# saithepaithewhyyy/Stochastic-Gradient-MCMC-for-non-linear-state-models---MTH422

Measured on AMD Instinct MI355X. Metric: SGLD steps/sec (T=1000, N=1000 particles), higher is better.
Workload: dtype f64

## Files before the change

stochastic-gradient-mcmc-for-non-linear-state-models---mth422_amd/csrc/pfg_launch.hpp:

```cpp
#pragma once
#include <mutex>
#include "pfg_host.hpp"
#include "pfg_device.hpp"

namespace pfg_host {

#define PFG_ENSURE_LDS(ctx, kern, lds)                                                                    \
    do {                                                                                                  \
        if ((lds) > 64 * 1024) {                                                                          \
            size_t &pfg_lds_set_ = (ctx)->lds_set[reinterpret_cast<const void *>(kern)];                  \
            if ((lds) > pfg_lds_set_) {                                                                   \
                PFG_HIP(ctx, hipFuncSetAttribute(reinterpret_cast<const void *>(kern),                    \
                                                 hipFuncAttributeMaxDynamicSharedMemorySize, (int)(lds))); \
                pfg_lds_set_ = (lds);                                                                     \
            }                                                                                             \
        }                                                                                                 \
    } while (0)

constexpr int PFG_GRID_ALL = -1, PFG_GRID_INIT = -2, PFG_GRID_FINISH = -3;
template <int MODEL, int KERNEL, typename REAL, int RNG, int NT, int PPT, int KMAX>
int launch_grid_ppt(pfg_ctx *ctx, const LaunchPlan &p, int B, const pfg_dev_problem *dp, hipStream_t st) {
    constexpr int NW = NT / pfg::WAVE;
    const int phase = p.phase;
    const dim3 grid((unsigned)p.tiles, (unsigned)B), blk(NT);
// ... 40 lines not shown
    PFG_HIP(ctx, hipGetLastError());
    return PFG_OK;
}


template <int TAG>
int ensure_exp_tab_mem(pfg_ctx *ctx, hipStream_t st) {
    static std::mutex mu;
    static std::vector<char> filled;
    std::lock_guard<std::mutex> lock(mu);
    if ((size_t)ctx->device < filled.size() && filled[(size_t)ctx->device]) return PFG_OK;
    hipStreamCaptureStatus cap = hipStreamCaptureStatusNone;
    PFG_HIP(ctx, hipStreamIsCapturing(st, &cap));
    if (cap != hipStreamCaptureStatusNone)
        return fail(ctx, PFG_ERR_INVALID, "the first launch of this kernel on a device fills its exp table and cannot be captured: run one eager launch first");
    hipLaunchKernelGGL(pfg::exp_tab_mem_fill_kernel<TAG>, dim3(1), dim3(pfg::TAB_E2_ACC), 0, st);
    PFG_HIP(ctx, hipGetLastError());
    PFG_HIP(ctx, hipStreamSynchronize(st));
    if (filled.size() <= (size_t)ctx->device) filled.resize((size_t)ctx->device + 1, 0);
    filled[(size_t)ctx->device] = 1;
    return PFG_OK;
}

template <int MODEL, int KERNEL, typename REAL, int NT, int PPT, int RNG, bool PP, int MODE, bool TRACE = true, bool SCORE1 = false>
int launch_one_t(pfg_ctx *ctx, const LaunchPlan &p, int B, const pfg_dev_problem *dp, hipStream_t st) {
    using TR = pfg::RegTraits<MODEL, KERNEL, REAL, NT, PPT, RNG, PP, MODE>;
    if constexpr (TR::TABMEM) {
        if (const int rc = ensure_exp_tab_mem<TR::EXPTAB_TAG>(ctx, st)) return rc;
    }
    return launch_kernel(ctx, pfg::pf_reg_kernel<MODEL, KERNEL, REAL, NT, PPT, RNG, PP, MODE, TRACE, SCORE1>, NT, p, B, dp, st);
}
template <int MODEL, int KERNEL, typename REAL, int NT, int PPT, int RNG, bool PP>
int launch_one(pfg_ctx *ctx, const LaunchPlan &p, int B, const pfg_dev_problem *dp, hipStream_t st) {
    if constexpr (reg_score1_twin(MODEL, RNG, sizeof(REAL) == 8, NT, PPT, PP))
        if (p.score1) return launch_one_t<MODEL, KERNEL, REAL, NT, PPT, RNG, PP, pfg::MODE_PLAIN, false, true>(ctx, p, B, dp, st);
    if (!p.traced) return launch_one_t<MODEL, KERNEL, REAL, NT, PPT, RNG, PP, pfg::MODE_PLAIN, false>(ctx, p, B, dp, st);
    return launch_one_t<MODEL, KERNEL, REAL, NT, PPT, RNG, PP, pfg::MODE_PLAIN, true>(ctx, p, B, dp, st);
}
template <int MODEL, int KERNEL, typename REAL, int RNG>
int launch_v(pfg_ctx *ctx, const LaunchPlan &p, int B, const pfg_dev_problem *dp, hipStream_t st) {
#define PFG_ENTRY(NT_, PPT_, PP_)                                                                 \
    if constexpr (reg_entry_built(MODEL, RNG, sizeof(REAL) == 8, NT_, PPT_, PP_))                \
        if (p.nt == NT_ && p.ppt == PPT_ && p.pp == PP_) return launch_one<MODEL, KERNEL, REAL, NT_, PPT_, RNG, PP_>(ctx, p, B, dp, st);
    PFG_ENTRY(256, 1, true) PFG_ENTRY(256, 4, true) PFG_ENTRY(256, 4, false) PFG_ENTRY(1024, 1, true) PFG_ENTRY(64, 2, true)
    PFG_ENTRY(1024, 4, false) PFG_ENTRY(64, 4, true) PFG_ENTRY(512, 2, false)
    PFG_ENTRY(64, 2, false) PFG_ENTRY(64, 4, false)
#undef PFG_ENTRY
    return fail(ctx, PFG_ERR_INVALID, "the launch plan names no kernel of this unit");
}

template <int MODEL, int KERNEL, typename REAL, int RNG, int MODE>
// ... 88 lines not shown
```

stochastic-gradient-mcmc-for-non-linear-state-models---mth422_amd/csrc/pfg_math.hpp:

```cpp
#pragma once
#include <hip/hip_runtime.h>
#include <stdint.h>
#include <type_traits>
#include "pfgrad.h"

namespace pfg {

constexpr int WAVE = 64;
constexpr int MODE_PLAIN = 0, MODE_PARIS = 1, MODE_SYSTEMATIC = 2, MODE_N2 = 3, MODE_STRATIFIED = 4, MODE_ADAPTIVE = 5;
__host__ __device__ inline float ess_threshold_of(int32_t reserved) { return __builtin_bit_cast(float, reserved); }
constexpr double LOG_2PI = 1.8378770664093453;

template <class T> using gptr = T __attribute__((address_space(1))) *;
template <class T> __device__ __forceinline__ gptr<T> global_ptr(T *p) { return (gptr<T>)p; }

template <int CTRL>
__device__ __forceinline__ double dpp_shr0_f64(double v) {
    int lo = __builtin_amdgcn_mov_dpp(__double2loint(v), CTRL, 0xf, 0xf, true);
    int hi = __builtin_amdgcn_mov_dpp(__double2hiint(v), CTRL, 0xf, 0xf, true);
    return __hiloint2double(hi, lo);
}
template <int CTRL, int ROW_MASK>
__device__ __forceinline__ double dpp_f64(double old, double v) {
    int lo = __builtin_amdgcn_update_dpp(__double2loint(old), __double2loint(v), CTRL, ROW_MASK, 0xf, false);
// ... 295 lines not shown
    }
    template <int HOT> __device__ __forceinline__ double exp_finite_hot(double x) const {
        if constexpr (HOT == 0) return exp_tab<true>(x, t.e2); else return exp_tab_hot<true, HOT>(x, t);
    }
#endif
#else
    __device__ __forceinline__ double exp_finite(double x) const { return exp_tab(x, t.e2); }
#endif
    __device__ __forceinline__ double log(double x) const { return log_tab(x, t.lg); }
    __device__ __forceinline__ double sqrt(double x) const { return ::sqrt(x); }
    __device__ __forceinline__ double sqrt_pos(double x) const { return pfg::sqrt_pos(x); }
    __device__ __forceinline__ double rcp_pos(double x) const { return pfg::rcp_pos(x); }
    __device__ __forceinline__ void normal_pair_f32(uint32_t a, uint32_t b, float &z0, float &z1) const {
        const float u1 = ((float)a + 0.5f) * 2.3283064365386963e-10f;
        const float u2 = (float)(b >> 8) * (1.0f / 16777216.0f);
        const float r = __builtin_amdgcn_sqrtf(-1.3862943611198906f * __builtin_amdgcn_logf(u1));
        z0 = r * __builtin_amdgcn_cosf(u2);
        z1 = r * __builtin_amdgcn_sinf(u2);
    }
    __device__ __forceinline__ void normal_pair(uint32_t a, uint32_t b, double &z0, double &z1) const {
        float f0, f1;
        normal_pair_f32(a, b, f0, f1);
        z0 = (double)f0; z1 = (double)f1;
    }
};
template <> struct Math<double, false> {
    TabF64 t;
    __device__ __forceinline__ double exp(double x) const { return ::exp(x); }
    __device__ __forceinline__ double exp_acc(double x) const { return ::exp(x); }
    __device__ __forceinline__ double exp_finite(double x) const { return ::exp(x); }
    __device__ __forceinline__ double log(double x) const { return ::log(x); }
    __device__ __forceinline__ double sqrt(double x) const { return ::sqrt(x); }
    __device__ __forceinline__ double sqrt_pos(double x) const { return ::sqrt(x); }
    __device__ __forceinline__ double rcp_pos(double x) const { return 1.0 / x; }
    __device__ __forceinline__ void normal_pair(uint32_t a, uint32_t b, double &z0, double &z1) const {
        const double u1 = ((double)a + 0.5) * (1.0 / 4294967296.0);
        const double r = ::sqrt(-2.0 * ::log(u1));
        double sn, cs;
        sincospi((double)b * (1.0 / 2147483648.0), &sn, &cs);
        z0 = r * cs; z1 = r * sn;
    }
    __device__ __forceinline__ void normal_pair_f32(uint32_t a, uint32_t b, float &z0, float &z1) const {
        double d0, d1;
        normal_pair(a, b, d0, d1);
        z0 = (float)d0; z1 = (float)d1;
    }
// ... 28 lines not shown
```

stochastic-gradient-mcmc-for-non-linear-state-models---mth422_amd/csrc/pfg_reg_kernel.hpp:

```cpp
#pragma once
#include "pfg_reg_traits.hpp"

namespace pfg {

template <int NW> __device__ __forceinline__ void block_sync() {
    if (NW == 1) {
        __builtin_amdgcn_fence(__ATOMIC_RELEASE, "wavefront");
        __builtin_amdgcn_wave_barrier();
        __builtin_amdgcn_fence(__ATOMIC_ACQUIRE, "wavefront");
    } else {
        __syncthreads();
    }
}
__device__ __forceinline__ double rcp_newton2(double x) {
    double r = __builtin_amdgcn_rcp(x);
    r = fma(fma(-x, r, 1.0), r, r);
    r = fma(fma(-x, r, 1.0), r, r);
    return r;
}

template <int MODEL, int KERNEL, typename REAL, int NT, int PPT, int RNG, bool PP, int MODE = 0, bool TRACE = true, bool SCORE1 = false>
__global__ __launch_bounds__(NT) __attribute__((amdgpu_waves_per_eu(RegTraits<MODEL, KERNEL, REAL, NT, PPT, RNG, PP, MODE>::OCC_MIN, RegTraits<MODEL, KERNEL, REAL, NT, PPT, RNG, PP, MODE>::OCC_MAX))) void pf_reg_kernel(const pfg_dev_problem *__restrict__ probs) {
    using TR = RegTraits<MODEL, KERNEL, REAL, NT, PPT, RNG, PP, MODE>;
    constexpr int NS = TR::NS, H = TR::H, NW = TR::NW;
    static_assert(!TR::LWL || PP, "PaRIS / O(N^2) need the parents intact while children are built: ping-pong buffers");
    static_assert(!TR::SYSTEMATIC || RNG == PFG_RNG_DEVICE, "systematic resampling draws its offset on the device");
    extern __shared__ __align__(16) unsigned char smem[];

    const pfg_dev_problem &P = probs[blockIdx.x];
    const int N = P.N, T = P.T, t1 = P.t1, tL = P.tL;
    const int tid = threadIdx.x, lane = tid & (WAVE - 1);
    const int wave = __builtin_amdgcn_readfirstlane(tid / WAVE);
    constexpr bool ONLY_SCORE1 = PFG_EXP_PLAIN || SCORE1;
    if constexpr (SCORE1) {
        if (P.smoother != PFG_SMOOTHER_NEMETH || P.lambduh != 1.0 || P.stat != PFG_STAT_SCORE) {
            if (threadIdx.x < PFG_OUT_DOUBLES && P.out) P.out[threadIdx.x] = __builtin_nan("");
            return;
        }
    }
    if constexpr (TR::ADAPTIVE) {
        if (!(P.flags & PFG_FLAG_ADAPTIVE_RESAMPLING) || P.smoother != PFG_SMOOTHER_NEMETH || P.stat == PFG_STAT_PREDICTIVE) {
            if (threadIdx.x < PFG_OUT_DOUBLES && P.out) P.out[threadIdx.x] = __builtin_nan("");
            return;
        }
    }
    [[maybe_unused]] const double tauN = TR::ADAPTIVE ? (double)ess_threshold_of(P.reserved) * (double)N : 0.0;
    const bool is_filter = !ONLY_SCORE1 && (P.smoother == PFG_SMOOTHER_FILTER);
    const int stat = ONLY_SCORE1 ? (int)PFG_STAT_SCORE : P.stat;
    const double lam_d = ONLY_SCORE1 ? 1.0 : is_filter ? 0.0 : ((P.smoother == PFG_SMOOTHER_PARIS || TR::N2) ? 1.0 : P.lambduh);
    const REAL lam = (REAL)lam_d, oml = (REAL)(1.0 - lam_d);
    const bool needS_every = is_filter || (lam_d != 1.0);
    [[maybe_unused]] const bool raw_score = TR::RAWSCORE && !needS_every && stat == PFG_STAT_SCORE;
    const gptr<const double> yv = global_ptr(P.y);
    const gptr<const double> wv = global_ptr(P.weights);
    const gptr<const double> uv = global_ptr(P.u);
    const gptr<const double> zv = global_ptr(P.z);

    const int NLS = TR::FAST ? TR::layout(0).NLS : TR::layout(N).NLS;
    double *cdf = reg_lds_ptr<double, TR, &RegLdsLayout::cdf>(smem, N);
    uint32_t *cdfu = reg_lds_ptr<uint32_t, TR, &RegLdsLayout::cdf>(smem, N);
    REAL *cur = reg_lds_ptr<REAL, TR, &RegLdsLayout::buf0>(smem, N), *nxt = reg_lds_ptr<REAL, TR, &RegLdsLayout::buf1>(smem, N);
    auto sidx = [&](int d, int i) -> size_t { return TR::sidx(NLS, d, i); };
    double *red_scan = reg_lds_ptr<double, TR, &RegLdsLayout::red_scan>(smem, N);
    double *red_max = reg_lds_ptr<double, TR, &RegLdsLayout::red_max>(smem, N);
    float *red_maxf = reinterpret_cast<float *>(red_max);
    double *red_S = reg_lds_ptr<double, TR, &RegLdsLayout::red_S>(smem, N);
    double *red_W0 = reg_lds_ptr<double, TR, &RegLdsLayout::red_W0>(smem, N);
    const double invN = 1.0 / (double)N;
    double *tabmem = reg_lds_ptr<double, TR, &RegLdsLayout::tab>(smem, N);
    REAL *lwL = reg_lds_ptr<REAL, TR, &RegLdsLayout::lwL>(smem, N);
    int *paris_queue = reg_lds_ptr<int, TR, &RegLdsLayout::queue>(smem, N);
    int *paris_wq0 = reg_lds_ptr<int, TR, &RegLdsLayout::wq0>(smem, N), *paris_wq1 = reg_lds_ptr<int, TR, &RegLdsLayout::wq1>(smem, N);
    int *paris_Jres = reg_lds_ptr<int, TR, &RegLdsLayout::Jres>(smem, N);

    Math<REAL, TR::TAB> mth;
    mth.t.e2 = tabmem;
    mth.t.lg = reinterpret_cast<const double2 *>(tabmem + TAB_E2);
    mth.t.sc = reinterpret_cast<const double2 *>(tabmem + TAB_E2 + 2 * TAB_LG);
    if constexpr (TR::TABMEM) mth.t.e2g = (gptr<const double>)ExpTabMem<TR::EXPTAB_TAG>::e2;
    if (tab_bytes<REAL, RNG, TR::TAB>() > 0) tab_fill(tabmem, RNG == PFG_RNG_DEVICE, tid, NT);
    if (TR::FAST && !TR::BLK) {
// ... 7 lines not shown
    int np2 = 1;
    while (np2 < N) np2 <<= 1;
    if (P.stamps && tid == 0) { P.stamps[0] = __builtin_amdgcn_s_memtime(); P.stamps[1] = __builtin_amdgcn_s_memrealtime(); }
#ifdef PFG_PHASE_STAMPS
    unsigned long long ph_acc[10] = {0, 0, 0, 0, 0, 0, 0, 0, 0, 0};
    unsigned long long ph_prev = __builtin_amdgcn_s_memtime();
#define PFG_PH(i) { const unsigned long long ph_now = __builtin_amdgcn_s_memtime(); ph_acc[i] += ph_now - ph_prev; ph_prev = ph_now; }
#define PFG_MARK(s)
#elif defined(PFG_ISA_MARKERS)
#define PFG_PH(i) asm volatile("; PFG_PHASE " #i);
#define PFG_MARK(s) asm volatile("; PFG_MARK " s);
#else
#define PFG_PH(i)
#define PFG_MARK(s)
#endif

    LaneRng rng = {};
    if (RNG == PFG_RNG_DEVICE)
        rng = lane_rng_init(P.seed, P.stream, P.step_ctr ? *P.step_ctr : 0ull, (uint32_t)tid);
    auto draw_normals = [&](REAL *zz) {
#pragma unroll
        for (int k = 0; k < PPT; k += 2) {
            REAL a, b;
            mth.normal_pair(rng.next(), rng.next(), a, b);
            zz[k] = a;
            if (k + 1 < PPT) zz[k + 1] = b;
        }
    };

    REAL lw[PPT];
    long long paris_cursor = 0;
    bool paris_overflow = false;
    const bool raw = TR::RAWCAP && (P.flags & PFG_FLAG_PARIS_RAW_STREAM) != 0 && P.paris_stream != nullptr;
    bool carry_has = false;
    double *const zbuf = reinterpret_cast<double *>(paris_queue);
    long long *const raw_slots = reinterpret_cast<long long *>(red_W0 + 2);
    [[maybe_unused]] auto legacy_normals = [&]() {
        const gptr<const double> strm = global_ptr(P.paris_stream);
        const long long cap = P.paris_stream_len;
        const unsigned long long ltm = (1ull << lane) - 1ull;
        int *const wc = reinterpret_cast<int *>(red_scan);
        const int produced0 = carry_has ? 1 : 0;
        __syncthreads();
        if (carry_has && tid == 0) zbuf[0] = red_W0[1];
        const int need = (N - produced0 + 1) >> 1;
        const long long base = paris_cursor;
        int acc = 0;
// ... 118 lines not shown
    for (int h = 0; h < H; ++h) { filt[h] = 0.0; S[h] = 0.0; }
    double m = 0.0, W = (double)N;
    bool valid[PPT];
    int own[PPT];
#pragma unroll
    for (int k = 0; k < PPT; ++k) {
        valid[k] = (k * NT + tid) < N;
        own[k] = valid[k] ? (k * NT + tid) : (N - 1);
        if (!valid[k]) lw[k] = -INFINITY;
    }
    const int last = N - 1;
    [[maybe_unused]] float m_next = 0.0f;
    if constexpr (TR::STALE) {
        float ml = (float)lw[0];
#pragma unroll
        for (int k = 1; k < PPT; ++k) ml = fmaxf(ml, (float)lw[k]);
        ml = wave_max(ml);
        if (lane == 0) red_maxf[wave] = ml;
        block_sync<NW>();
        float mm = red_maxf[0];
#pragma unroll
        for (int w = 1; w < NW; ++w) mm = fmaxf(mm, red_maxf[w]);
        m = uniform_f64((double)mm);
        block_sync<NW>();
        if constexpr (TR::SHIFTFOLD) {
#pragma unroll
            for (int k = 0; k < PPT; ++k) lw[k] -= (REAL)m;
        }
    }

    for (int t = 0; t <= T; ++t) {
        [[maybe_unused]] double uu_raw[PPT];
        [[maybe_unused]] REAL zz_raw[PPT];
        if constexpr (TR::RAWCAP) {
            if (raw && t < T) {
                const gptr<const double> strm = global_ptr(P.paris_stream);
                if (paris_cursor + N > P.paris_stream_len) paris_overflow = true;
#pragma unroll
                for (int k = 0; k < PPT; ++k) uu_raw[k] = paris_overflow ? 0.5 : strm[paris_cursor + own[k]];
                if (!paris_overflow) paris_cursor += N;
                legacy_normals();
#pragma unroll
                for (int k = 0; k < PPT; ++k) zz_raw[k] = (REAL)zbuf[own[k]];
            }
        }
        [[maybe_unused]] float ml = 0.0f;
// ... 96 lines not shown
        PFG_PH(3)
        if (TR::BLK && NW == 1) {
            W = __hiloint2double(__builtin_amdgcn_readlane(__double2hiint(wave_inc), WAVE - 1),
                                 __builtin_amdgcn_readlane(__double2loint(wave_inc), WAVE - 1));
        } else if (TR::BLK) {
            const double tot = (lane < NW) ? red_scan[lane] : 0.0;
            double inc = tot;
            inc += dpp_shr0_f64<0x111>(inc);
            inc += dpp_shr0_f64<0x112>(inc);
            if (NW > 4) { inc += dpp_shr0_f64<0x114>(inc); inc += dpp_shr0_f64<0x118>(inc); }
            const double exc = inc - tot;
            const double off = __hiloint2double(__builtin_amdgcn_readlane(__double2hiint(exc), wave),
                                                __builtin_amdgcn_readlane(__double2loint(exc), wave));
#pragma unroll
            for (int k = 0; k < PPT; ++k) cs[k] += off;
            W = __hiloint2double(__builtin_amdgcn_readlane(__double2hiint(inc), NW - 1),
                                 __builtin_amdgcn_readlane(__double2loint(inc), NW - 1));
            if constexpr (TR::STALE) {
                bool retry;
                if constexpr (TR::SUMSHIFT) {
                    constexpr uint32_t W_LO = (uint32_t)(1023 - 728) << 20, W_HI = (uint32_t)(1023 + 728) << 20;
                    retry = t > 0 && !((uint32_t)__double2hiint(W) - W_LO < W_HI - W_LO);
                } else {
                    float mm = red_maxf[0];
#pragma unroll
                    for (int w = 1; w < NW; ++w) mm = fmaxf(mm, red_maxf[w]);
                    if constexpr (TR::SHIFTFOLD) mm += (float)m;
                    m_next = __builtin_bit_cast(float, __builtin_amdgcn_readfirstlane(__builtin_bit_cast(int, mm)));
                    retry = t > 0 && !(fabsf(m_next - (float)m) <= 512.0f);
                }
                if (retry) {
                    PFG_MARK("cold stale-shift-retry")
                    block_sync<NW>();
                    if constexpr (!TR::SUMSHIFT) m = uniform_f64((double)m_next);
                    const REAL y_p = (REAL)yv[t - 1], y2_p = y_p * y_p;
                    REAL lwk[PPT];
#pragma unroll
                    for (int k = 0; k < PPT; ++k) {
                        const REAL x1 = cur[sidx(0, own[k])];
                        lwk[k] = valid[k] ? svm_logw(c, x1, mth.exp_finite(-x1), y2_p) : (REAL)(-INFINITY);
                        if constexpr (!TR::SUMSHIFT) cs[k] = (double)mth.exp((REAL)(lwk[k] - (REAL)m));
                    }
                    if constexpr (TR::SUMSHIFT) {
                        float rl = (float)lwk[0];
#pragma unroll
                        for (int k = 1; k < PPT; ++k) rl = fmaxf(rl, (float)lwk[k]);
                        rl = wave_max(rl);
                        if (lane == 0) red_maxf[wave] = rl;
                        block_sync<NW>();
                        float mm = red_maxf[0];
#pragma unroll
                        for (int w = 1; w < NW; ++w) mm = fmaxf(mm, red_maxf[w]);
                        m = uniform_f64((double)mm);
#pragma unroll
                        for (int k = 0; k < PPT; ++k) cs[k] = (double)mth.exp((REAL)(lwk[k] - (REAL)m));
                    }
                    if constexpr (TR::SHIFTFOLD) {
// ... 82 lines not shown
            }
            W = uniform_f64(run);
        }
        const double invW = uniform_f64(PFG_OPT_RCPW ? rcp_newton2(W) : 1.0 / W);
        [[maybe_unused]] bool resample = true;
        if constexpr (TR::ADAPTIVE) {
            if (t < T) {
                double W2 = red_W0[4];
#pragma unroll
                for (int w = 1; w < NW; ++w) W2 += red_W0[4 + w];
                resample = __builtin_amdgcn_readfirstlane((int)(W * W < tauN * W2)) != 0;
            }
        }
        if (needS) {
            PFG_MARK("cold needS")
#pragma unroll
            for (int h = 0; h < H; ++h) {
                double acc = 0.0;
#pragma unroll
                for (int w = 0; w < NW; ++w) acc += red_S[h * NW + w];
                S[h] = uniform_f64(acc * invW);
            }
        }
        if (wave == 0) {
            PFG_MARK("w0.25 wave0-loglik")
            const bool counts = t > 0 && (t - 1) >= t1 && (t - 1) < tL;
            if (TR::LAZYLL) {
                const bool mine = lane == (t & (WAVE - 1));
                ll_W = mine ? W : ll_W;
                ll_w = mine ? (counts ? wt_prev : 0.0) : ll_w;
                ll_m = mine ? (float)m : ll_m;
                const bool due = (t & (WAVE - 1)) == WAVE - 1 || t == T;
                if (due || (!TR::TWINLESS_LL && PFG_TR(P.trace_ll))) {
                    PFG_MARK("cold loglik-flush")
                    const double term = ll_w * ((double)ll_m + (double)mth.log((REAL)(ll_W * invN)));
                    ll = uniform_f64(ll + wave_sum(term));
                    ll_w = 0.0;
                } else if (TR::TWINLESS_LL && PFG_TR(P.trace_ll)) {
                    const double term = ll_w * ((double)ll_m + (double)mth.log((REAL)(ll_W * invN)));
                    const double run = ll + wave_sum(term);
                    if (tid == 0) P.trace_ll[t] = run;
                }
                if ((due || !TR::TWINLESS_LL) && PFG_TR(P.trace_ll) && tid == 0) P.trace_ll[t] = ll;
            } else {
                if (counts) ll = uniform_f64(ll + wt_prev * (m + log(W / (double)N)));
                if (PFG_TR(P.trace_ll) && tid == 0) P.trace_ll[t] = ll;
            }
// ... 12 lines not shown
        const bool use_stat = inside && (stat != PFG_STAT_NONE);
        const bool plain = !needS_every;
        if (!TR::ADAPTIVE || resample) {
        if (TR::BLK) {
            {
                const double fixs = invW * 4294967296.0;
#pragma unroll
                for (int k = 0; k < PPT; ++k)
                    cdfu[cdf_phys(tid * PPT + k)] = cvt_u32_sat(cs[k] * fixs);
            }
        } else {
#pragma unroll
            for (int k = 0; k < PPT; ++k)
                if (valid[k]) {
                    cdf[TR::FAST ? cdf_phys(k * NT + tid) : k * NT + tid] = cs[k] * invW;
                    if (TR::PARIS || TR::N2) lwL[k * NT + tid] = lw[k];
                }
        }
        PFG_PH(4)
        block_sync<NW>();
        PFG_PH(5)
        if (TR::PRIO == 1) __builtin_amdgcn_s_setprio(2);
        if (TR::PRIO == 2) __builtin_amdgcn_s_setprio(0);

        if (RNG != PFG_RNG_REPLAY) {
            if (TR::SYSTEMATIC) {
                const double u0 = red_W0[0];
#pragma unroll
                for (int k = 0; k < PPT; ++k) uu[k] = ((double)(k * NT + tid) + u0) * invN;
                if (PFG_TR(P.trace_x) && P.rec_ud) {
#pragma unroll
                    for (int k = 0; k < PPT; ++k)
                        if (valid[k]) P.rec_ud[(size_t)t * N + k * NT + tid] = uu[k];
                }
            } else if (TR::STRATIFIED) {
#pragma unroll
                for (int k = 0; k < PPT; ++k) uu[k] = ((double)(k * NT + tid) + u01_32(rng.next())) * invN;
                if (PFG_TR(P.trace_x) && P.rec_ud) {
#pragma unroll
                    for (int k = 0; k < PPT; ++k)
                        if (valid[k]) P.rec_ud[(size_t)t * N + k * NT + tid] = uu[k];
                }
            } else if (!TR::BLK) {
#pragma unroll
                for (int k = 0; k < PPT; ++k) uu[k] = u01_32(rng.next());
                if (TR::ADAPTIVE && PFG_TR(P.trace_x) && P.rec_ud) {
// ... 6 lines not shown
#pragma unroll
            for (int k = 0; k < PPT; ++k) uu[k] = ((double)(k * NT + tid) + uu[k]) / (double)N;
        }
        }
        int anc[PPT];
        [[maybe_unused]] uint32_t gaddr[PPT];
#pragma unroll
        for (int k = 0; k < PPT; ++k) { anc[k] = 0; gaddr[k] = 0u; }
        if (!TR::ADAPTIVE || resample) {
        if (TR::BLK) {
            uint32_t ua[PPT];
#pragma unroll
            for (int k = 0; k < PPT; ++k) ua[k] = TR::SORTED ? us[k] : rng.next();
#ifdef PFG_EXP_EVENWORDS
#pragma unroll
            for (int k = 0; k < PPT; ++k) ua[k] = (uint32_t)(((uint64_t)(tid * PPT + k) << 32) / (uint64_t)(NT * PPT)) + (ua[k] >> 12);
#endif
            if (PFG_TR(P.trace_x) && P.rec_u) {
#pragma unroll
                for (int k = 0; k < PPT; ++k)
                    if (valid[k]) P.rec_u[(size_t)t * N + k * NT + tid] = ua[k];
            }
            using lds_u32 = const __attribute__((address_space(3))) uint32_t;
            const uint32_t cdf_base = (uint32_t)(uintptr_t)(lds_u32 *)cdfu;
            uint32_t off[PPT];
#pragma unroll
            for (int k = 0; k < PPT; ++k) off[k] = cdf_base;
            constexpr int FIRST_STEP = TR::PIVOTS ? 128 : (NT * PPT) >> 1;
            if constexpr (TR::PIVOTS) {
                const uint32_t p511 = __builtin_amdgcn_readfirstlane(cdfu[cdf_phys(511)]);
                const uint32_t p255 = __builtin_amdgcn_readfirstlane(cdfu[cdf_phys(255)]);
                const uint32_t p767 = __builtin_amdgcn_readfirstlane(cdfu[cdf_phys(767)]);
#pragma unroll
                for (int k = 0; k < PPT; ++k) {
                    const bool g1 = p511 <= ua[k];
                    const uint32_t t2 = g1 ? p767 : p255;
                    const bool g2 = t2 <= ua[k];
                    off[k] += (g1 ? 4u * (512 + 16) : 0u) + (g2 ? 4u * (256 + 8) : 0u);
                }
            }
#pragma unroll
            for (int step = FIRST_STEP; step >= 1; step >>= 1) {
                const int probe = step - 1 + (step >= 32 ? (step >> 5) - 1 : 0);
                const int adv = step + (step >> 5);
                uint32_t cv[PPT];
#pragma unroll
                for (int k = 0; k < PPT; ++k) cv[k] = *(lds_u32 *)(uintptr_t)(off[k] + 4u * probe);
// ... 84 lines not shown
        } else {
#pragma unroll
            for (int k = 0; k < PPT; ++k) { anc[k] = (TR::FAST || valid[k]) ? k * NT + tid : last; gaddr[k] = 0u; }
        }
        [[maybe_unused]] double lse = 0.0, lgN = 0.0;
        if constexpr (TR::ADAPTIVE) {
            if (!resample) { lse = uniform_f64(log(W)); lgN = uniform_f64(log((double)N)); }
        }
        PFG_PH(6)
        auto slots = [&](auto stat_tag) {
            constexpr int STAT = decltype(stat_tag)::value;
            if (STAT != PFG_STAT_SCORE) { PFG_MARK("cold sufficient-statistics") }
            REAL xp[PPT][NS], sp[PPT][H];
#pragma unroll
            for (int k = 0; k < PPT; ++k) {
                if constexpr (TR::PAIRED) {
                    typedef double dv2 __attribute__((ext_vector_type(2)));
                    REAL rec[NS + H];
#pragma unroll
                    for (int p = 0; p < (NS + H) / 2; ++p) {
                        dv2 v;
                        if constexpr (TR::GADDR) {
                            using lds_byte = const __attribute__((address_space(3))) unsigned char;
                            v = *(const __attribute__((address_space(3))) dv2 *)((lds_byte *)cur + gaddr[k] + (uint32_t)(p * 16 * NLS));
                        } else {
                            v = *reinterpret_cast<const dv2 *>(&cur[sidx(2 * p, anc[k])]);
                        }
                        rec[2 * p] = (REAL)v.x; rec[2 * p + 1] = (REAL)v.y;
                    }
#pragma unroll
                    for (int d = 0; d < NS; ++d) xp[k][d] = rec[d];
#pragma unroll
                    for (int h = 0; h < H; ++h) sp[k][h] = rec[NS + h];
                } else {
#pragma unroll
                for (int d = 0; d < NS; ++d) xp[k][d] = cur[sidx(d, anc[k])];
#pragma unroll
                for (int h = 0; h < H; ++h) sp[k][h] = cur[sidx((NS + h), anc[k])];
                }
            }
            PFG_PH(7)
            if (TR::PRIO == 1) __builtin_amdgcn_s_setprio(0);
            if (TR::PRIO == 2) __builtin_amdgcn_s_setprio(2);
            if (!PP && (!TR::ADAPTIVE || resample)) block_sync<NW>();
            PFG_PH(8)
            if (RNG != PFG_RNG_REPLAY) {
// ... 9 lines not shown
            if constexpr (TR::SHIFTFOLD) k0_shifted = (REAL)uniform_f64((double)(c.c0 + c.logLRinv) - m);
#endif
            auto children = [&](auto upd_tag) {
                constexpr int UPD = decltype(upd_tag)::value;
                constexpr bool RAWUPD = TR::RAWSCORE && STAT == PFG_STAT_SCORE && UPD == 0;
                [[maybe_unused]] constexpr int TUNE = RAWUPD ? TR::STEP_TUNE : (TR::STEP_TUNE & ~PFG_STEP_RAWSCORE);
                if (UPD == 1) { PFG_MARK("cold children-outside-window") }
                if (UPD == 2) { PFG_MARK("cold children-general") }
#pragma unroll
                for (int k = 0; k < PPT; ++k) {
                    REAL xn[NS], add[H], lwn;
#ifdef PFG_FAST_ALGEBRA
#if PFG_OPT_SHIFTFOLD
                    if constexpr (TR::STEP_TUNE != 0) particle_step_svm_tuned<STAT, TUNE>(c, mth, xp[k], (REAL)y_t, zz[k], xn, lwn, add, k0_shifted);
#else
                    if constexpr (TR::STEP_TUNE != 0) particle_step_svm_tuned<STAT, TUNE>(c, mth, xp[k], (REAL)y_t, zz[k], xn, lwn, add, (REAL)0);
#endif
                    else
#endif
                    particle_step<MODEL, KERNEL, STAT, REAL>(c, mth, xp[k], (REAL)y_t, zz[k], xn, lwn, add);
                    if constexpr (TR::ADAPTIVE) {
                        if (!resample) lwn = (REAL)(((((double)lw[k] - m) - lse) + lgN) + (double)lwn);
                    }
                    lw[k] = valid[k] ? lwn : (REAL)(-INFINITY);
                    if constexpr (RAWUPD) {
                        const REAL y2 = (REAL)y_t * (REAL)y_t, wy2 = (REAL)wt * y2;
                        const REAL zw = (REAL)wt * add[1];
                        sp[k][0] = fma(wy2, add[0], sp[k][0]);
                        sp[k][1] = fma(zw, add[1], sp[k][1]);
                        sp[k][2] = fma(zw, add[2], sp[k][2]);
                    } else if (UPD == 0) {
#pragma unroll
                        for (int h = 0; h < H; ++h) sp[k][h] = sp[k][h] + add[h] * (REAL)wt;
                    } else if (UPD == 2) {
#pragma unroll
                        for (int h = 0; h < H; ++h) {
                            const REAL a = use_stat ? add[h] * (REAL)wt : (REAL)0;
                            const REAL sm = (lam * sp[k][h] + oml * (REAL)S[h]) + a;
                            sp[k][h] = is_filter ? a : sm;
                        }
                    }
                    if ((TR::FAST && NT < 1024) || valid[k]) {
                        const int i = k * NT + tid;
                        if constexpr (TR::PAIRED) {
                            typedef double dv2 __attribute__((ext_vector_type(2)));
                            REAL rec[NS + H];
#pragma unroll
                            for (int d = 0; d < NS; ++d) rec[d] = xn[d];
#pragma unroll
                            for (int h = 0; h < H; ++h) rec[NS + h] = sp[k][h];
#pragma unroll
                            for (int p = 0; p < (NS + H) / 2; ++p) {
                                dv2 v;
                                v.x = (double)rec[2 * p]; v.y = (double)rec[2 * p + 1];
                                *reinterpret_cast<dv2 *>(&nxt[sidx(2 * p, i)]) = v;
                            }
                        } else {
#pragma unroll
                        for (int d = 0; d < NS; ++d) nxt[sidx(d, i)] = xn[d];
#pragma unroll
                        for (int h = 0; h < H; ++h) nxt[sidx((NS + h), i)] = sp[k][h];
                        }
                    }
                }
            };
            if (!plain) children(std::integral_constant<int, 2>{});
            else if (use_stat) children(std::integral_constant<int, 0>{});
            else children(std::integral_constant<int, 1>{});
        };
        auto paris_slots = [&](auto stat_tag) {
            constexpr int STAT = decltype(stat_tag)::value;
            const int Nt = P.Ntilde, R = P.max_accept_reject;
            const double *__restrict__ const pidx = P.paris_idx_u;
            const double *__restrict__ const pacc = P.paris_acc_u;
            const double *__restrict__ const pman = P.paris_man_u;
            int *queue = paris_queue;
            int *qcount = reinterpret_cast<int *>(red_max) + NW;
// ... 424 lines not shown
                    for (int d = 0; d < NS; ++d) P.trace_x[row * NS + d] = (double)nxt[sidx(d, i)];
                    P.trace_logw[row] = TR::SHIFTFOLD ? (double)lw[k] + m : (double)lw[k];
                    if (P.trace_stats && !is_filter) {
                        if constexpr (TR::RAWSCORE) {
                            REAL r[H], sv[H];
#pragma unroll
                            for (int h = 0; h < H; ++h) r[h] = sv[h] = nxt[sidx((NS + h), i)];
                            if (raw_score) raw_score_out(c, (REAL)Cw, r, sv);
#pragma unroll
                            for (int h = 0; h < H; ++h) P.trace_stats[row * H + h] = (double)sv[h];
                        } else {
#pragma unroll
                        for (int h = 0; h < H; ++h)
                            P.trace_stats[row * H + h] = (double)nxt[sidx((NS + h), i)];
                        }
                    }
                }
            }
        }
        if (PP) { REAL *tmp = cur; cur = nxt; nxt = tmp; }
        wt_prev = wt;
        PFG_PH(9)
    }
    if (P.stamps && tid == 0) { P.stamps[2] = __builtin_amdgcn_s_memtime(); P.stamps[3] = __builtin_amdgcn_s_memrealtime(); }
#ifdef PFG_PHASE_STAMPS
    if (P.stamps && lane == 0) {
#pragma unroll
        for (int q = 0; q < 10; ++q) atomicAdd(reinterpret_cast<unsigned long long *>(P.stamps) + 4 + q, ph_acc[q]);
    }
#endif
#undef PFG_PH
#undef PFG_MARK

    if (RNG == PFG_RNG_REPLAY && P.out) {
        tie = -wave_max(-tie);
        if (lane == 0) red_max[wave] = tie;
        __syncthreads();
        tie = red_max[0];
#pragma unroll
        for (int w = 1; w < NW; ++w) tie = red_max[w] < tie ? red_max[w] : tie;
    }
    if (TR::PARIS && tid == 0 && P.paris_consumed) {
        P.paris_consumed[0] = paris_overflow ? -1ll : paris_cursor;
        P.paris_consumed[1] = (TR::RAWCAP && raw && carry_has && !paris_overflow) ? paris_cursor - raw_slots[1] : 0ll;
    }
    if constexpr (TR::RAWSCORE) {
// ... 48 lines not shown
```

stochastic-gradient-mcmc-for-non-linear-state-models---mth422_amd/csrc/pfg_reg_traits.hpp:

```cpp
#pragma once
#include "pfg_models.hpp"

namespace pfg {

#ifndef PFG_OPT_PADSTATE
#define PFG_OPT_PADSTATE 1
#endif
#ifndef PFG_OCC64
#define PFG_OCC64 4
#endif
#ifndef PFG_OCC4
#define PFG_OCC4 1
#endif
#ifndef PFG_OPT_SORTED1024
#define PFG_OPT_SORTED1024 1
#endif
#ifndef PFG_OPT_PRIO
#define PFG_OPT_PRIO 1
#endif
#ifndef PFG_OPT_PAIRSTATE
#define PFG_OPT_PAIRSTATE 1
#endif
#ifndef PFG_OPT_STALESHIFT
#define PFG_OPT_STALESHIFT 1
#endif
#ifndef PFG_OPT_GATHERADDR
#define PFG_OPT_GATHERADDR 1
#endif
#ifndef PFG_OPT_SUMSHIFT
#define PFG_OPT_SUMSHIFT 0
#endif
#ifndef PFG_OPT_SHIFTFOLD
#define PFG_OPT_SHIFTFOLD 0
#endif
#ifndef PFG_OPT_SCOREDZ
#define PFG_OPT_SCOREDZ 1
#endif
#ifndef PFG_OPT_RAWSCORE
#define PFG_OPT_RAWSCORE 1
#endif
#ifndef PFG_OPT_EXPTABMEM
#define PFG_OPT_EXPTABMEM 0
#endif
#ifndef PFG_OPT_EXPMAGIC
#define PFG_OPT_EXPMAGIC 1
#endif
#ifndef PFG_OPT_N2SKIP
#define PFG_OPT_N2SKIP 1
#endif
#define PFG_TR(p) (TRACE && (p))
#ifndef PFG_EXP_PLAIN
#define PFG_EXP_PLAIN 0
#endif
#ifdef PFG_EXP_TABLANE
#define PFG_TABLANE_ON 1
#else
#define PFG_TABLANE_ON 0
#endif
#ifdef PFG_EXP_OWNGATHER
#define PFG_GATHERADDR_ON 0
#else
#define PFG_GATHERADDR_ON PFG_OPT_GATHERADDR
#endif
#ifdef PFG_FAST_ALGEBRA
#ifndef PFG_OPT_LAZYLL
#define PFG_OPT_LAZYLL 1
#endif
#ifndef PFG_OPT_RCPW
// ... 36 lines not shown

template <int MODEL, int KERNEL, typename REAL, int NT, int PPT, int RNG, bool PP, int MODE = MODE_PLAIN>
struct RegTraits {
    static constexpr int NS = ModelDims<MODEL>::NS, H = ModelDims<MODEL>::H;
    static constexpr int NW = NT / WAVE, SLOTS = NT * PPT;
    static constexpr bool PARIS = MODE == MODE_PARIS, N2 = MODE == MODE_N2, SYSTEMATIC = MODE == MODE_SYSTEMATIC;
    static constexpr bool STRATIFIED = MODE == MODE_STRATIFIED;
    static constexpr bool ADAPTIVE = MODE == MODE_ADAPTIVE;
    static_assert(!ADAPTIVE || NT / WAVE <= 4, "the per-wave sums of w^2 sit in red_W0[4 .. 4 + NW)");
    static constexpr bool LWL = PARIS || N2;
    static constexpr bool FAST = PP || NT <= 512 || NT == 1024;
    static constexpr bool TAB = FAST;
    static constexpr bool BLK = FAST && RNG == PFG_RNG_DEVICE && MODE == MODE_PLAIN && (PPT & (PPT - 1)) == 0;
    static constexpr int LOG_PPT = PPT == 1 ? 0 : (PPT == 2 ? 1 : (PPT == 4 ? 2 : (PPT == 8 ? 3 : 4)));
    static_assert(PPT <= 16, "LOG_PPT covers 1, 2, 4, 8, 16 particles per thread");
    static constexpr bool SORTED = PFG_OPT_SORTED1024 && BLK && NT == 1024 && PPT == 4 && !SYSTEMATIC && NW > 1;
    static constexpr int PRIO = !(PFG_OPT_PRIO && (BLK || (RNG == PFG_RNG_REPLAY && MODE == MODE_PLAIN)) && !PP && PPT == 4) ? 0
                                : (NT == 1024 ? 1 : (NT == 256 ? 2 : 0));
    static constexpr bool PAIRED = PFG_OPT_PAIRSTATE && BLK && sizeof(REAL) == 8 && ((NS + H) % 2 == 0);
    static constexpr bool STALE = PFG_OPT_STALESHIFT && BLK && MODEL == PFG_MODEL_SVM && KERNEL == PFG_KERNEL_PRIOR && NT == 256 && PPT == 4 &&
                                  !PP && sizeof(REAL) == 8;
    static constexpr bool SUMSHIFT = PFG_OPT_SUMSHIFT && STALE, SHIFTFOLD = PFG_OPT_SHIFTFOLD && STALE, SCOREDZ = PFG_OPT_SCOREDZ && STALE;
    static constexpr bool RAWSCORE = PFG_OPT_RAWSCORE && STALE;
#ifdef PFG_HAS_EXP_HOT
    static constexpr bool TABMEM_B = (PFG_OPT_EXPTABMEM & 1) && STALE, TABMEM_G = (PFG_OPT_EXPTABMEM & 2) && STALE, EXPMAGIC = PFG_OPT_EXPMAGIC && STALE;
    static constexpr int HOT_COMMON = (EXPMAGIC ? PFG_HOT_MAGIC : 0) | ((PFG_TABLANE_ON && STALE) ? PFG_HOT_LANE : 0);
    static constexpr int HOT_B = HOT_COMMON | (TABMEM_B ? PFG_HOT_MEM : 0), HOT_G = HOT_COMMON | (TABMEM_G ? PFG_HOT_MEM : 0);
#else
    static constexpr bool TABMEM_B = false, TABMEM_G = false, EXPMAGIC = false;
    static constexpr int HOT_B = 0, HOT_G = 0;
#endif
    static constexpr bool TABMEM = TABMEM_B || TABMEM_G;
    static constexpr int EXPTAB_TAG = MODEL * 16 + KERNEL;
    static constexpr int STEP_TUNE = (SHIFTFOLD ? PFG_STEP_SHIFTFOLD : 0) | (SCOREDZ ? PFG_STEP_SCOREDZ : 0) | (RAWSCORE ? PFG_STEP_RAWSCORE : 0) |
                                     (HOT_G << PFG_STEP_HOT_SHIFT);
    static constexpr bool GADDR = PFG_GATHERADDR_ON && BLK && PAIRED && NT == 256 && PPT == 4 && MODEL == PFG_MODEL_SVM && !PP;
    static_assert(!GADDR || 4 * (SLOTS + SLOTS / 32) * 993 < (1 << 23), "GADDR: rel * 993 must fit the 24-bit multiply");
    static constexpr bool LAZYLL = PFG_OPT_LAZYLL && TAB && sizeof(REAL) == 8;
    static constexpr bool TWINLESS_LL = STRATIFIED || N2 || ADAPTIVE || PARIS || SYSTEMATIC;
    static constexpr bool PIVOTS = PFG_OPT_PIVOTS && SLOTS == 1024;
    static constexpr bool RAWCAP = MODE == MODE_PARIS && RNG == PFG_RNG_REPLAY;

    static constexpr bool OCC_LDS4096 = SLOTS == 4096 && NT < 1024;
    static constexpr bool OCC_TWO = MODEL == PFG_MODEL_GARCH && sizeof(REAL) == 8 && NT == 256 && PPT == 4 && !PP;
    static constexpr bool OCC_DEV4 = PFG_OCC4 && MODEL == PFG_MODEL_SVM && NT == 256 && PPT == 4 && !PP && RNG == PFG_RNG_DEVICE && MODE == MODE_PLAIN;
    static constexpr int OCC_MAX = OCC_TWO ? 2 : OCC_LDS4096 ? (NT == 512 ? 2 : 1) : NT == 64 ? PFG_OCC64
                                   : (NT >= 512 || PPT == 1 || OCC_DEV4) ? 4 : ((PP && sizeof(REAL) == 8) ? 2 : 3);
    static constexpr int OCC_MIN = OCC_TWO ? 2 : OCC_LDS4096 ? (NT == 512 ? 2 : 1)
                                   : NT == 512 ? 4
                                   : OCC_DEV4 ? 4 : ((NT == 256 && PPT == 4 && !PP) ? 3 : 1);

    __device__ __forceinline__ static size_t sidx(int NLS, int d, int i) {
        return PAIRED ? (size_t)(d >> 1) * (2 * (size_t)NLS) + 2 * (size_t)i + (size_t)(d & 1) : (size_t)d * NLS + (size_t)i;
    }

    static constexpr int RED_SCAN = PPT * NW, RED_MAX = NW, RED_S = PFG_MAX_STAT * NW, RED_W0 = 8;
    static_assert(sizeof(int) * (NW + 1) <= sizeof(double) * RED_MAX, "the queue count fits behind red_maxf");
    __host__ __device__ static constexpr RegLdsLayout layout(int N) {
        RegLdsLayout L = {};
        L.NL = FAST ? SLOTS : (N + WAVE - 1) / WAVE * WAVE;
        L.NLS = L.NL + ((PFG_OPT_PADSTATE && FAST && RNG == PFG_RNG_DEVICE) ? (int)(8 / sizeof(REAL)) : 0);
// ... 35 lines not shown
```

Baseline: 304,400.

## Add trimmed normal sampling, hi-word masking, deferred loglik and absolute LDS addressing

Adds four compile-time options to the STALE register kernel path. TRIM (on by default) folds the uniform offset into an FMA in the Box-Muller sampler and computes the four-wave max with v_max3 inline asm. HIMASK (on by default) masks invalid log-weights by overwriting only the high word instead of a full select. LLBEHIND (defers the wave-0 log-likelihood accumulation into a lagged per-lane buffer) and LDSABS (addresses LDS from absolute layout offsets, with a host check that no static LDS precedes it) are off by default.

Result: no change. 306,400, median of 6 (+0.6%).

```diff
diff --git a/stochastic-gradient-mcmc-for-non-linear-state-models---mth422_amd/csrc/pfg_launch.hpp b/stochastic-gradient-mcmc-for-non-linear-state-models---mth422_amd/csrc/pfg_launch.hpp
--- a/stochastic-gradient-mcmc-for-non-linear-state-models---mth422_amd/csrc/pfg_launch.hpp
+++ b/stochastic-gradient-mcmc-for-non-linear-state-models---mth422_amd/csrc/pfg_launch.hpp
@@ -1,4 +1,5 @@
 #pragma once
+#include <atomic>
 #include <mutex>
 #include "pfg_host.hpp"
 #include "pfg_device.hpp"
@@ -86,11 +87,30 @@
     return PFG_OK;
 }
 
+template <pf_kernel_t KERN>
+struct DynamicLdsAtZero { static inline std::atomic<int> state{0}; };
+template <pf_kernel_t KERN>
+int ensure_dynamic_lds_at_zero(pfg_ctx *ctx) {
+    int s = DynamicLdsAtZero<KERN>::state.load(std::memory_order_acquire);
+    if (s == 0) {
+        hipFuncAttributes attr = {};
+        PFG_HIP(ctx, hipFuncGetAttributes(&attr, reinterpret_cast<const void *>(KERN)));
+        s = attr.sharedSizeBytes == 0 ? 1 : -1;
+        DynamicLdsAtZero<KERN>::state.store(s, std::memory_order_release);
+    }
+    if (s < 0)
+        return fail(ctx, PFG_ERR_UNSUPPORTED, "this kernel addresses its dynamic LDS from 0 (PFG_OPT_LDSABS) but was built with static LDS in front of it: rebuild with -DPFG_OPT_LDSABS=0");
+    return PFG_OK;
+}
+
 template <int MODEL, int KERNEL, typename REAL, int NT, int PPT, int RNG, bool PP, int MODE, bool TRACE = true, bool SCORE1 = false>
 int launch_one_t(pfg_ctx *ctx, const LaunchPlan &p, int B, const pfg_dev_problem *dp, hipStream_t st) {
     using TR = pfg::RegTraits<MODEL, KERNEL, REAL, NT, PPT, RNG, PP, MODE>;
     if constexpr (TR::TABMEM) {
         if (const int rc = ensure_exp_tab_mem<TR::EXPTAB_TAG>(ctx, st)) return rc;
+    }
+    if constexpr (TR::LDSABS) {
+        if (const int rc = ensure_dynamic_lds_at_zero<pfg::pf_reg_kernel<MODEL, KERNEL, REAL, NT, PPT, RNG, PP, MODE, TRACE, SCORE1>>(ctx)) return rc;
     }
     return launch_kernel(ctx, pfg::pf_reg_kernel<MODEL, KERNEL, REAL, NT, PPT, RNG, PP, MODE, TRACE, SCORE1>, NT, p, B, dp, st);
 }
diff --git a/stochastic-gradient-mcmc-for-non-linear-state-models---mth422_amd/csrc/pfg_math.hpp b/stochastic-gradient-mcmc-for-non-linear-state-models---mth422_amd/csrc/pfg_math.hpp
--- a/stochastic-gradient-mcmc-for-non-linear-state-models---mth422_amd/csrc/pfg_math.hpp
+++ b/stochastic-gradient-mcmc-for-non-linear-state-models---mth422_amd/csrc/pfg_math.hpp
@@ -341,6 +341,13 @@
         float f0, f1;
         normal_pair_f32(a, b, f0, f1);
         z0 = (double)f0; z1 = (double)f1;
+    }
+    __device__ __forceinline__ void normal_pair_ufma(uint32_t a, uint32_t b, double &z0, double &z1) const {
+        const float u1 = __builtin_fmaf((float)a, 2.3283064365386963e-10f, 1.1641532182693481e-10f);
+        const float u2 = (float)(b >> 8) * (1.0f / 16777216.0f);
+        const float r = __builtin_amdgcn_sqrtf(-1.3862943611198906f * __builtin_amdgcn_logf(u1));
+        z0 = (double)(r * __builtin_amdgcn_cosf(u2));
+        z1 = (double)(r * __builtin_amdgcn_sinf(u2));
     }
 };
 template <> struct Math<double, false> {
diff --git a/stochastic-gradient-mcmc-for-non-linear-state-models---mth422_amd/csrc/pfg_reg_kernel.hpp b/stochastic-gradient-mcmc-for-non-linear-state-models---mth422_amd/csrc/pfg_reg_kernel.hpp
--- a/stochastic-gradient-mcmc-for-non-linear-state-models---mth422_amd/csrc/pfg_reg_kernel.hpp
+++ b/stochastic-gradient-mcmc-for-non-linear-state-models---mth422_amd/csrc/pfg_reg_kernel.hpp
@@ -17,6 +17,21 @@
     r = fma(fma(-x, r, 1.0), r, r);
     r = fma(fma(-x, r, 1.0), r, r);
     return r;
+}
+
+template <typename MATH>
+__device__ __forceinline__ void ll_behind(const MATH &mth, const pfg_dev_problem &P, int t, int T, int t1, int tL, int lane, int tid, bool traced,
+                                          double W, double wt_prev, double invN, double &ll, double &ll_W, double &ll_w, float ll_m) {
+    const bool counts = t > 0 && (t - 1) >= t1 && (t - 1) < tL;
+    const bool mine = lane == (t & (WAVE - 1));
+    ll_W = mine ? W : ll_W;
+    ll_w = mine ? (counts ? wt_prev : 0.0) : ll_w;
+    if ((t & (WAVE - 1)) == WAVE - 1 || t == T || traced) {
+        const double term = ll_w * ((double)ll_m + mth.log(ll_W * invN));
+        ll = uniform_f64(ll + wave_sum(term));
+        ll_w = 0.0;
+    }
+    if (traced && tid == 0) P.trace_ll[t] = ll;
 }
 
 template <int MODEL, int KERNEL, typename REAL, int NT, int PPT, int RNG, bool PP, int MODE = 0, bool TRACE = true, bool SCORE1 = false>
@@ -57,6 +72,8 @@
     const gptr<const double> zv = global_ptr(P.z);
 
     const int NLS = TR::FAST ? TR::layout(0).NLS : TR::layout(N).NLS;
+    constexpr bool HIMASK = TR::HIMASK && !TRACE, TRIM = TR::TRIM && !TRACE;
+    [[maybe_unused]] constexpr RegLdsLayout LAY0 = TR::layout(0);
     double *cdf = reg_lds_ptr<double, TR, &RegLdsLayout::cdf>(smem, N);
     uint32_t *cdfu = reg_lds_ptr<uint32_t, TR, &RegLdsLayout::cdf>(smem, N);
     REAL *cur = reg_lds_ptr<REAL, TR, &RegLdsLayout::buf0>(smem, N), *nxt = reg_lds_ptr<REAL, TR, &RegLdsLayout::buf1>(smem, N);
@@ -110,7 +127,8 @@
 #pragma unroll
         for (int k = 0; k < PPT; k += 2) {
             REAL a, b;
-            mth.normal_pair(rng.next(), rng.next(), a, b);
+            if constexpr (TRIM) mth.normal_pair_ufma(rng.next(), rng.next(), a, b);
+            else mth.normal_pair(rng.next(), rng.next(), a, b);
             zz[k] = a;
             if (k + 1 < PPT) zz[k + 1] = b;
         }
@@ -275,6 +293,7 @@
 #pragma unroll
         for (int w = 1; w < NW; ++w) mm = fmaxf(mm, red_maxf[w]);
         m = uniform_f64((double)mm);
+        if constexpr (TR::LLBEHIND) ll_m = mm;
         block_sync<NW>();
         if constexpr (TR::SHIFTFOLD) {
 #pragma unroll
@@ -417,9 +436,15 @@
                     constexpr uint32_t W_LO = (uint32_t)(1023 - 728) << 20, W_HI = (uint32_t)(1023 + 728) << 20;
                     retry = t > 0 && !((uint32_t)__double2hiint(W) - W_LO < W_HI - W_LO);
                 } else {
-                    float mm = red_maxf[0];
+                    float mm;
+                    if constexpr (TRIM && NW == 4) {
+                        const float r0 = red_maxf[0], r1 = red_maxf[1], r2 = red_maxf[2], r3 = red_maxf[3];
+                        asm("v_max3_f32 %0, %1, %2, %3\n\tv_max_f32_e32 %0, %0, %4" : "=&v"(mm) : "v"(r0), "v"(r1), "v"(r2), "v"(r3));
+                    } else {
+                    mm = red_maxf[0];
 #pragma unroll
                     for (int w = 1; w < NW; ++w) mm = fmaxf(mm, red_maxf[w]);
+                    }
                     if constexpr (TR::SHIFTFOLD) mm += (float)m;
                     m_next = __builtin_bit_cast(float, __builtin_amdgcn_readfirstlane(__builtin_bit_cast(int, mm)));
                     retry = t > 0 && !(fabsf(m_next - (float)m) <= 512.0f);
@@ -428,6 +453,7 @@
                     PFG_MARK("cold stale-shift-retry")
                     block_sync<NW>();
                     if constexpr (!TR::SUMSHIFT) m = uniform_f64((double)m_next);
+                    if constexpr (TR::LLBEHIND) ll_m = lane == (t & (WAVE - 1)) ? m_next : ll_m;
                     const REAL y_p = (REAL)yv[t - 1], y2_p = y_p * y_p;
                     REAL lwk[PPT];
 #pragma unroll
@@ -556,7 +582,7 @@
                 S[h] = uniform_f64(acc * invW);
             }
         }
-        if (wave == 0) {
+        if (wave == 0 && !TR::LLBEHIND) {
             PFG_MARK("w0.25 wave0-loglik")
             const bool counts = t > 0 && (t - 1) >= t1 && (t - 1) < tL;
             if (TR::LAZYLL) {
@@ -615,6 +641,13 @@
         PFG_PH(5)
         if (TR::PRIO == 1) __builtin_amdgcn_s_setprio(2);
         if (TR::PRIO == 2) __builtin_amdgcn_s_setprio(0);
+        if constexpr (TR::LLBEHIND) {
+            if (wave == 0) {
+                PFG_MARK("w0.25 wave0-loglik")
+                ll_behind(mth, P, t, T, t1, tL, lane, tid, PFG_TR(P.trace_ll), W, wt_prev, invN, ll, ll_W, ll_w, ll_m);
+                ll_m = lane == ((t + 1) & (WAVE - 1)) ? (float)m : ll_m;
+            }
+        }
 
         if (RNG != PFG_RNG_REPLAY) {
             if (TR::SYSTEMATIC) {
@@ -667,7 +700,7 @@
                     if (valid[k]) P.rec_u[(size_t)t * N + k * NT + tid] = ua[k];
             }
             using lds_u32 = const __attribute__((address_space(3))) uint32_t;
-            const uint32_t cdf_base = (uint32_t)(uintptr_t)(lds_u32 *)cdfu;
+            const uint32_t cdf_base = TR::LDSABS ? (uint32_t)LAY0.cdf : (uint32_t)(uintptr_t)(lds_u32 *)cdfu;
             uint32_t off[PPT];
 #pragma unroll
             for (int k = 0; k < PPT; ++k) off[k] = cdf_base;
@@ -798,6 +831,9 @@
                         dv2 v;
                         if constexpr (TR::GADDR) {
                             using lds_byte = const __attribute__((address_space(3))) unsigned char;
+                            if constexpr (TR::LDSABS)
+                                v = *(const __attribute__((address_space(3))) dv2 *)(uintptr_t)((uint32_t)LAY0.buf0 + gaddr[k] + (uint32_t)(p * 16 * NLS));
+                            else
                             v = *(const __attribute__((address_space(3))) dv2 *)((lds_byte *)cur + gaddr[k] + (uint32_t)(p * 16 * NLS));
                         } else {
                             v = *reinterpret_cast<const dv2 *>(&cur[sidx(2 * p, anc[k])]);
@@ -853,6 +889,9 @@
                     if constexpr (TR::ADAPTIVE) {
                         if (!resample) lwn = (REAL)(((((double)lw[k] - m) - lse) + lgN) + (double)lwn);
                     }
+                    if constexpr (HIMASK) {
+                        lw[k] = (REAL)__hiloint2double(valid[k] ? __double2hiint((double)lwn) : (int)0xFFE00000u, __double2loint((double)lwn));
+                    } else
                     lw[k] = valid[k] ? lwn : (REAL)(-INFINITY);
                     if constexpr (RAWUPD) {
                         const REAL y2 = (REAL)y_t * (REAL)y_t, wy2 = (REAL)wt * y2;
@@ -884,6 +923,9 @@
                             for (int p = 0; p < (NS + H) / 2; ++p) {
                                 dv2 v;
                                 v.x = (double)rec[2 * p]; v.y = (double)rec[2 * p + 1];
+                                if constexpr (TR::LDSABS)
+                                    *(__attribute__((address_space(3))) dv2 *)(uintptr_t)((uint32_t)LAY0.buf1 + 8u * (uint32_t)sidx(2 * p, i)) = v;
+                                else
                                 *reinterpret_cast<dv2 *>(&nxt[sidx(2 * p, i)]) = v;
                             }
                         } else {
@@ -1354,6 +1396,9 @@
         wt_prev = wt;
         PFG_PH(9)
     }
+    if constexpr (TR::LLBEHIND) {
+        if (wave == 0) ll_behind(mth, P, T, T, t1, tL, lane, tid, PFG_TR(P.trace_ll), W, wt_prev, invN, ll, ll_W, ll_w, ll_m);
+    }
     if (P.stamps && tid == 0) { P.stamps[2] = __builtin_amdgcn_s_memtime(); P.stamps[3] = __builtin_amdgcn_s_memrealtime(); }
 #ifdef PFG_PHASE_STAMPS
     if (P.stamps && lane == 0) {
diff --git a/stochastic-gradient-mcmc-for-non-linear-state-models---mth422_amd/csrc/pfg_reg_traits.hpp b/stochastic-gradient-mcmc-for-non-linear-state-models---mth422_amd/csrc/pfg_reg_traits.hpp
--- a/stochastic-gradient-mcmc-for-non-linear-state-models---mth422_amd/csrc/pfg_reg_traits.hpp
+++ b/stochastic-gradient-mcmc-for-non-linear-state-models---mth422_amd/csrc/pfg_reg_traits.hpp
@@ -44,6 +44,18 @@
 #endif
 #ifndef PFG_OPT_EXPMAGIC
 #define PFG_OPT_EXPMAGIC 1
+#endif
+#ifndef PFG_OPT_LLBEHIND
+#define PFG_OPT_LLBEHIND 0
+#endif
+#ifndef PFG_OPT_LDSABS
+#define PFG_OPT_LDSABS 0
+#endif
+#ifndef PFG_OPT_HIMASK
+#define PFG_OPT_HIMASK 1
+#endif
+#ifndef PFG_OPT_TRIM
+#define PFG_OPT_TRIM 1
 #endif
 #ifndef PFG_OPT_N2SKIP
 #define PFG_OPT_N2SKIP 1
@@ -126,6 +138,8 @@
                                   !PP && sizeof(REAL) == 8;
     static constexpr bool SUMSHIFT = PFG_OPT_SUMSHIFT && STALE, SHIFTFOLD = PFG_OPT_SHIFTFOLD && STALE, SCOREDZ = PFG_OPT_SCOREDZ && STALE;
     static constexpr bool RAWSCORE = PFG_OPT_RAWSCORE && STALE;
+    static constexpr bool LLBEHIND_ASKED = PFG_OPT_LLBEHIND && STALE && !(PFG_OPT_SUMSHIFT || PFG_OPT_SHIFTFOLD), HIMASK = PFG_OPT_HIMASK && STALE;
+    static constexpr bool TRIM = PFG_OPT_TRIM && STALE;
 #ifdef PFG_HAS_EXP_HOT
     static constexpr bool TABMEM_B = (PFG_OPT_EXPTABMEM & 1) && STALE, TABMEM_G = (PFG_OPT_EXPTABMEM & 2) && STALE, EXPMAGIC = PFG_OPT_EXPMAGIC && STALE;
     static constexpr int HOT_COMMON = (EXPMAGIC ? PFG_HOT_MAGIC : 0) | ((PFG_TABLANE_ON && STALE) ? PFG_HOT_LANE : 0);
@@ -141,6 +155,8 @@
     static constexpr bool GADDR = PFG_GATHERADDR_ON && BLK && PAIRED && NT == 256 && PPT == 4 && MODEL == PFG_MODEL_SVM && !PP;
     static_assert(!GADDR || 4 * (SLOTS + SLOTS / 32) * 993 < (1 << 23), "GADDR: rel * 993 must fit the 24-bit multiply");
     static constexpr bool LAZYLL = PFG_OPT_LAZYLL && TAB && sizeof(REAL) == 8;
+    static constexpr bool LLBEHIND = LLBEHIND_ASKED && LAZYLL;
+    static constexpr bool LDSABS = PFG_OPT_LDSABS && STALE && GADDR && FAST;
     static constexpr bool TWINLESS_LL = STRATIFIED || N2 || ADAPTIVE || PARIS || SYSTEMATIC;
     static constexpr bool PIVOTS = PFG_OPT_PIVOTS && SLOTS == 1024;
     static constexpr bool RAWCAP = MODE == MODE_PARIS && RNG == PFG_RNG_REPLAY;
```
